# ds4dm/Tulip.jl

Hardware: AMD Instinct MI355X
Metric: IPM Newton-step rate: KKT.update! (A*D*A'+Rd, supernodal Cholesky) + 4 KKT.solve! (higher is better)
Workload: dtype f64

## Files before the change

### tulip.jl_amd/csrc/kernels.hip

```cpp
#include <hip/hip_runtime.h>

#include <algorithm>
#include <cstdlib>
#include <mutex>

#include "tlpk_device.hpp"

namespace tlpk {


typedef double v4f64 __attribute__((ext_vector_type(4)));
__device__ __forceinline__ double readlane_f64(const double v, const int l) {
    const int lo = __builtin_amdgcn_readlane(__double2loint(v), l), hi = __builtin_amdgcn_readlane(__double2hiint(v), l);
    return __hiloint2double(hi, lo);
}

__device__ __forceinline__ double *front_u(const DevCtx &c, const FrontDesc &fd) {
    return (fd.ubuf ? c.U1 : c.U0) + fd.uoff;
}
__device__ __forceinline__ double *pcol(const DevCtx &c, const FrontDesc &fd, i32 col) { return c.Lval + fd.loff + pk_off(fd.lda, col); }
__device__ __forceinline__ i32 pld(const FrontDesc &fd, i32 col) { return fd.lda - ((col >> 6) << 6); }
__device__ __forceinline__ bool front_skipped(const DevCtx &c, i32 front) { return c.front_skip != nullptr && c.front_skip[front] != 0; }
__device__ __forceinline__ void record_fail(const DevCtx &c, i32 col) {
    atomicMin(c.info, col);
// ... 129 lines not shown
                if (((tc - t.j0) & 3) != wave) continue;
                const double *__restrict__ src = Uc + (i64)q * rsc;
                double *__restrict__ dst = (tc < ns) ? pcol(c, fd, tc) : (Up + (i64)(tc - ns) * rs - ns);
                for (i32 r = max(q, rlo) + lane; r < rhi; r += 256) {
                    i32 tg[4]; double v[4], d[4];
#pragma unroll
                    for (int u = 0; u < 4; ++u) {
                        const i32 ru = min(r + 64 * u, rhi - 1);
                        tg[u] = relc[ru]; v[u] = src[ru];
                    }
#pragma unroll
                    for (int u = 0; u < 4; ++u) d[u] = dst[tg[u]];
#pragma unroll
                    for (int u = 0; u < 4; ++u) if (r + 64 * u < rhi) dst[tg[u]] = d[u] + v[u];
                }
            }
        }
    }
}

constexpr int EG_LD = EG_CAP_MAX / 64, EG_EB = 8, EG_CH = 2;
struct EgBatch { const i32 *rl[EG_EB]; const double *sr[EG_EB]; i32 n[EG_EB]; };
__device__ __forceinline__ EgBatch eg_entries(const DevCtx &c, const i64 e, const i64 e1) {
    EgBatch b;
#pragma unroll
    for (int u = 0; u < EG_EB; ++u) {
        const EaGatherEnt g = c.eg_ent[min(e + u, e1 - 1)];
        b.rl[u] = c.rel + g.rel;
        b.sr[u] = (((g.src >> EG_UBUF_BIT) & 1) ? c.U1 : c.U0) + (g.src & (((i64)1 << EG_UBUF_BIT) - 1));
        b.n[u] = (e + u < e1) ? g.n : 0;
    }
    return b;
}
__device__ __forceinline__ i32 eg_nmax(const EgBatch &b) {
    i32 m = 0;
#pragma unroll
    for (int u = 0; u < EG_EB; ++u) m = max(m, b.n[u]);
    return m;
}
__global__ __launch_bounds__(256, 4) void k_ea_gather(const EaTask *__restrict__ tasks, DevCtx c, int slice_rows) {
    extern __shared__ double eg_slices[];
    const EaTask t = tasks[blockIdx.x];
    if (!ea_task_gathered(c, t) || front_skipped(c, t.front)) return;
    const FrontDesc fd = c.fronts[t.front];
    const i32 f = fd.f, ns = fd.ns, rs = f - ns, cap = c.eg_cap;
    const int lane = threadIdx.x & 63;
    const int wave = __builtin_amdgcn_readfirstlane(threadIdx.x >> 6);
    double *slice = eg_slices + (size_t)wave * slice_rows;
    const i64 *colseg = c.eg_col + c.eg_base[t.front];
    double *Up = front_u(c, fd);
    for (i32 tc = t.j0 + wave; tc < t.j1; tc += 4) {
        double *__restrict__ col0 = (tc < ns) ? pcol(c, fd, tc) : (Up + (i64)(tc - ns) * rs - ns);
        const i64 g0 = colseg[tc], g1 = colseg[tc + 1];
        for (i64 g = g0; g < g1; ++g) {
            const i64 e0 = c.eg_ptr[g], e1 = c.eg_ptr[g + 1];
            if (e0 == e1) continue;
            const i32 r0 = tc + (i32)(g - g0) * cap, n = min(cap, f - r0);
            if (n > slice_rows) continue;
            double *__restrict__ col = col0 + r0;
            EgBatch b = eg_entries(c, e0, e1);
            double cv[EG_LD];
#pragma unroll
            for (int u = 0; u < EG_LD; ++u) cv[u] = col[min(lane + 64 * u, n - 1)];
            bool seeded = false;
            for (i64 e = e0; e < e1; e += EG_EB) {
                const bool thin = eg_nmax(b) <= 64 * EG_CH;
                i32 tg[EG_EB][EG_CH]; double v[EG_EB][EG_CH];
                if (thin) {
#pragma unroll
                    for (int u = 0; u < EG_EB; ++u)
#pragma unroll
                        for (int k = 0; k < EG_CH; ++k) {
                            const i32 ru = max(min(lane + 64 * k, b.n[u] - 1), 0);
                            tg[u][k] = b.rl[u][ru] - r0; v[u][k] = b.sr[u][ru];
                        }
                }
                if (!seeded) {
#pragma unroll
                    for (int u = 0; u < EG_LD; ++u) if (lane + 64 * u < n) slice[lane + 64 * u] = cv[u];
                    seeded = true;
                }
                EgBatch nb = b;
                if (e + EG_EB < e1) nb = eg_entries(c, e + EG_EB, e1);
                __builtin_amdgcn_wave_barrier();
                if (thin) {
#pragma unroll
                    for (int u = 0; u < EG_EB; ++u) {
                        double d[EG_CH];
#pragma unroll
                        for (int k = 0; k < EG_CH; ++k) d[k] = slice[tg[u][k]];
#pragma unroll
                        for (int k = 0; k < EG_CH; ++k) if (lane + 64 * k < b.n[u]) slice[tg[u][k]] = d[k] + v[u][k];
                        __builtin_amdgcn_wave_barrier();
                    }
                } else {
                    for (int u = 0; u < EG_EB; ++u) {
                        const i32 nu = b.n[u];
                        for (i32 r = lane; r - lane < nu; r += 256) {
                            i32 tq[4]; double w[4], d[4];
#pragma unroll
                            for (int k = 0; k < 4; ++k) { const i32 ru = min(r + 64 * k, nu - 1); tq[k] = b.rl[u][ru] - r0; w[k] = b.sr[u][ru]; }
#pragma unroll
                            for (int k = 0; k < 4; ++k) d[k] = slice[tq[k]];
#pragma unroll
                            for (int k = 0; k < 4; ++k) if (r + 64 * k < nu) slice[tq[k]] = d[k] + w[k];
                            __builtin_amdgcn_wave_barrier();
                        }
                    }
                }
                b = nb;
            }
            __builtin_amdgcn_wave_barrier();
            for (i32 r = lane; r < n; r += 64) col[r] = slice[r];
            __builtin_amdgcn_wave_barrier();
        }
    }
// ... 3417 lines not shown
    if (nrhs == 2) {
        if (L.kind == LK_FWD_SWEEP) {
            if (sw && L.pad) hipLaunchKernelGGL((k_fwd_sweep<2, true>), g, dim3(256), 0, st, a.fwd_sweep_tasks + L.first, a.ctx, *sw);
            else if (sw) hipLaunchKernelGGL(k_fwd_sweep<2>, g, dim3(256), 0, st, a.fwd_sweep_tasks + L.first, a.ctx, *sw);
            return;
        }
        if (L.kind == LK_BWD_SWEEP) {
            if (sw && L.pad) hipLaunchKernelGGL((k_bwd_sweep<2, true>), g, dim3(256), 0, st, a.bwd_sweep_tasks + L.first, a.ctx, *sw);
            else if (sw) hipLaunchKernelGGL(k_bwd_sweep<2>, g, dim3(256), 0, st, a.bwd_sweep_tasks + L.first, a.ctx, *sw);
            return;
        }
        const dim3 g2((unsigned)L.count, 2u);
        switch (L.kind) {
        case LK_FWD_GATHER: hipLaunchKernelGGL(k_fwd_gather, g2, dim3(256), 0, st, a.fwd_gather_tasks + L.first, a.ctx); return;
        case LK_FWD_SMALL: hipLaunchKernelGGL(k_fwd_small, g2, dim3(256), 0, st, a.fwd_small_tasks + L.first, a.ctx); return;
        case LK_BWD_SMALL: hipLaunchKernelGGL(k_bwd_small, g2, dim3(256), 0, st, a.bwd_small_tasks + L.first, a.ctx); return;
        default: break;
        }
        launch_tasks(st, a, L, sw, 1);
        DevArrays b = a;
        b.ctx.xw += a.ctx.xw2; b.ctx.uc += a.ctx.uc2;
        launch_tasks(st, b, L, sw, 1);
        return;
    }
#define TLPK_LAUNCH_S(KERNEL, TASKS) do { if (sgn) hipLaunchKernelGGL(KERNEL<true>, g, dim3(256), 0, st, TASKS + L.first, a.ctx); \
                                          else hipLaunchKernelGGL(KERNEL<false>, g, dim3(256), 0, st, TASKS + L.first, a.ctx); } while (0)
    switch (L.kind) {
    case LK_EXTEND_ADD: {
        static const unsigned ea_lds = [] { const char *e = std::getenv("TLPK_EA_LDS"); return e ? (unsigned)std::atoi(e) : 0u; }();
        bool plain = true;
        if (a.eg_launch) {
            const EaGatherLaunch *e = std::lower_bound(a.eg_launch, a.eg_launch + a.n_eg_launch, L.first, [](const EaGatherLaunch &x, i64 first) { return x.first < first; });
            if (e != a.eg_launch + a.n_eg_launch && e->first == L.first) {
                if (e->n_gather > 0)
                    hipLaunchKernelGGL(k_ea_gather, g, dim3(256), (unsigned)(4 * 8 * e->rows), st, a.ea_tasks + L.first, a.ctx, (int)e->rows);
                plain = e->n_plain > 0;
            }
        }
        if (plain) hipLaunchKernelGGL(k_extend_add, g, dim3(256), ea_lds, st, a.ea_tasks + L.first, a.ctx);
        break;
    }
    case LK_FRONT_ASSEMBLE:
        hipLaunchKernelGGL(k_front_assemble, g, dim3(256), 0, st, a.fa_tasks + L.first, a.ctx, a.asm_colptr, a.asm_target, a.asm_diag, a.asm_ptr,
                           a.pair_w, a.pair_j, a.asm_D, a.asm_regD);
        break;
    case LK_POTRF: case LK_POTRF_WIDE: {
        auto mode = [] {
            const char *m = std::getenv("TLPK_POTRF_MODE"); if (m) return std::atoi(m) & 3;
            const char *w = std::getenv("TLPK_POTRF_WAVE"); if (w && std::atoi(w) != 0) return 1;
            const char *e = std::getenv("TLPK_POTRF_PAIR"); if (e) return std::atoi(e) == 0 ? 0 : 2;
            return 3;
        };
        const bool dyn = std::getenv("TLPK_POTRF_DYN") != nullptr;
        static const int pm0 = mode();
        const int pm = dyn ? mode() : pm0;
#define TLPK_LAUNCH_PM(KERNEL, SG) do { if (pm == 3) hipLaunchKernelGGL((KERNEL<SG, 3>), g, dim3(256), 0, st, a.potrf_tasks + L.first, a.ctx); \
                                        else if (pm == 1) hipLaunchKernelGGL((KERNEL<SG, 1>), g, dim3(256), 0, st, a.potrf_tasks + L.first, a.ctx); \
                                        else if (pm == 2) hipLaunchKernelGGL((KERNEL<SG, 2>), g, dim3(256), 0, st, a.potrf_tasks + L.first, a.ctx); \
                                        else hipLaunchKernelGGL((KERNEL<SG, 0>), g, dim3(256), 0, st, a.potrf_tasks + L.first, a.ctx); } while (0)
#define TLPK_LAUNCH_P(KERNEL) do { if (sgn) TLPK_LAUNCH_PM(KERNEL, true); else TLPK_LAUNCH_PM(KERNEL, false); } while (0)
        if (L.kind == LK_POTRF) TLPK_LAUNCH_P(k_potrf); else TLPK_LAUNCH_P(k_potrf_wide);
#undef TLPK_LAUNCH_PM
#undef TLPK_LAUNCH_P
        break;
    }
    case LK_POTRF_SMALL: TLPK_LAUNCH_S(k_potrf_small, a.potrf_tasks); break;
    case LK_TRSM: TLPK_LAUNCH_S(k_trsm, a.trsm_tasks); break;
    case LK_TRSM_THIN: TLPK_LAUNCH_S(k_trsm_thin, a.trsm_tasks); break;
// ... 164 lines not shown
```

### tulip.jl_amd/csrc/symbolic.cpp

```cpp
#include "tlpk_host.hpp"
#include "schedule.hpp"
#include "../../include/tlpk.h"

#include <algorithm>
#include <atomic>
#include <thread>
#include <chrono>
#include <cstdio>
#include <array>
#include <cstdio>
#include <cstdlib>
#include <cstring>
#include <numeric>
#include <mutex>
#include <functional>
#include <condition_variable>
#include <map>
#include <climits>

namespace tlpk {

static inline i32 fa_min_f() {
    static const i32 v = [] { const char *e = std::getenv("TLPK_FA_MIN_F"); const int c = e ? std::atoi(e) : 0; return (i32)(c <= 0 ? INT32_MAX : c); }();
    return v;
// ... 1171 lines not shown
                i64 acc = 0;
                for (i64 e = a; e < b; ++e) { acc += S.pair_ptr[(size_t)e + 1]; S.pair_ptr[(size_t)e + 1] = acc; }
                tot[(size_t)ch + 1] = acc;
            });
            for (i64 ch = 0; ch < nch; ++ch) tot[(size_t)ch + 1] += tot[(size_t)ch];
            ok = ok && parallel_for(nch, host_threads(nch), [&](unsigned, i64 ch) {
                const i64 a = ch * CH, b = std::min(S.nnzS, a + CH), add = tot[(size_t)ch];
                if (add) for (i64 e = a; e < b; ++e) S.pair_ptr[(size_t)e + 1] += add;
            });
            if (!ok) return fail(S, TLPK_OOM, "out of memory while building the assembly lists");
            S.pair_ptr[0] = 0;
        }
        pt.mark("assembly lists: place");
        {
            S.pair_w.resize((size_t)S.pair_ptr[S.nnzS]); S.pair_j.resize((size_t)S.pair_ptr[S.nnzS]);
            const bool ok = parallel_for(m, host_threads(m / 256 + 1), [&](unsigned, i64 kk) {
                const i32 th = col_thr[(size_t)kk];
                if (th < 0) return;
                const i64 a = S.pair_ptr[(size_t)S.Sp[kk]], cnt = S.pair_ptr[(size_t)S.Sp[kk + 1]] - a;
                if (cnt <= 0) return;
                std::memcpy(S.pair_w.data() + a, st[(size_t)th].w.data() + col_off[(size_t)kk], (size_t)cnt * sizeof(double));
                std::memcpy(S.pair_j.data() + a, st[(size_t)th].j.data() + col_off[(size_t)kk], (size_t)cnt * sizeof(i32));
            }, 256);
            if (!ok) return fail(S, TLPK_OOM, "out of memory while building the assembly lists");
        }
    }
    pt.mark("schedule");
    S.error.clear();
    S.shared_device = opt.shared_device;
    build_schedule(S);
    if (!S.error.empty()) return TLPK_INTERNAL;
    for (const UpdateTask &u : S.update_tasks)
        if ((u.k0 & 15) != 0) return fail(S, TLPK_INTERNAL, "update task: K range does not start on a multiple of 16 columns");
    pt.mark(nullptr);
    return TLPK_OK;
}

int analyse(Symbolic &S, i64 m, i64 n, const i64 *colptr, const i64 *rowval, const double *nzval, int base, const Options &opt) {
    const int rc = analyse_common(S, m, n, colptr, rowval, nzval, base, opt);
    return rc != TLPK_OK ? rc : analyse_rank(S, opt);
}

int analyse_k2_common(Symbolic &S, i64 m, i64 n, const i64 *colptr, const i64 *rowval, const double *nzval,
                      int base, const Options &opt_in, Options *opt_out) {
    if (m < 0 || n < 0 || (base != 0 && base != 1) || !colptr) return fail(S, TLPK_BADARG, "bad dimensions or index base");
    if (opt_in.ordering == TLPK_ORDER_USER) return fail(S, TLPK_BADARG, "user_perm is not supported for K2");
    const i64 nnz = colptr[n] - base;
    if (nnz < 0 || m + n >= ((i64)1 << 31) || nnz >= ((i64)1 << 30)) return fail(S, TLPK_TOO_LARGE, "augmented system exceeds int32");
    if (nnz > 0 && (!rowval || !nzval)) return fail(S, TLPK_BADARG, "null rowval/nzval");
    std::vector<i64> bp((size_t)nnz + 1), bi((size_t)(2 * nnz));
    std::vector<double> bx((size_t)(2 * nnz));
    for (i64 j = 0; j < n; ++j) {
        if (colptr[j] - base < 0 || colptr[j + 1] < colptr[j] || colptr[j + 1] - base > nnz) return fail(S, TLPK_BADARG, "colptr not monotone");
        for (i64 p = colptr[j] - base; p < colptr[j + 1] - base; ++p) {
            const i64 r = rowval[p] - base;
            if (r < 0 || r >= m) return fail(S, TLPK_BADARG, "row index out of range");
            bp[(size_t)p] = 2 * p;
            bi[(size_t)(2 * p)] = j; bx[(size_t)(2 * p)] = 1.0;
            bi[(size_t)(2 * p + 1)] = n + r; bx[(size_t)(2 * p + 1)] = nzval[p];
        }
    }
    bp[(size_t)nnz] = 2 * nnz;
    Options opt = opt_in;
    opt.system = 1; opt.k2_n = n;
    std::vector<i64> node_block;
    if (opt_in.row_block) {
// ... 309 lines not shown
```

### tulip.jl_amd/csrc/tlpk_api.cpp

```cpp
#include <hip/hip_runtime.h>

#include <dlfcn.h>

#include <algorithm>
#include <atomic>
#include <chrono>
#include <climits>
#include <cmath>
#include <limits>
#include <cstdio>
#include <cstdlib>
#include <cstring>
#include <new>
#include <optional>
#include <string>
#include <thread>
#include <utility>
#include <vector>
#include <condition_variable>
#include <functional>
#include <initializer_list>
#include <mutex>

#include "../../include/tlpk.h"
// ... 156 lines not shown
        Launch cur = L[i];
        if ((h->profile || h->serial) && cur.kind == LK_UPDATE) {
            if (skip_update == i) continue;
            if (cur.side) {
                for (size_t j = i + 1; j < to && L[j].kind != LK_SIDE_JOIN; ++j)
                    if (L[j].kind == LK_UPDATE && !L[j].side && L[j].first == cur.first + cur.count) {
                        cur.count += L[j].count; skip_update = j; break;
                    }
            }
        }
        const bool stag = h->stagger && dir < 0 && !h->profile && !h->serial && cur.kind == LK_EXTEND_ADD && h->S.ngroups >= 2 && h->ev_stagger;
        if (stag && L[i].group == 1 && h->stagger_armed) { hipStreamWaitEvent(st, h->ev_stagger, 0); h->stagger_armed = false; }
        ProfScope ps(h, kind_class(cur.kind), st, &cur);
        if (stag && L[i].group == 0 && cur.count >= h->stagger_min) {
            launch_tasks(st, h->d, cur, nullptr, nrhs);
            hipEventRecord(h->ev_stagger, st); h->stagger_armed = true;
            continue;
        }
        if (cur.kind == LK_FWD_SWEEP || cur.kind == LK_BWD_SWEEP) {
            const i32 slot = (dir == 0 ? h->sweep_slot_fwd : h->sweep_slot_bwd)[i];
            SweepArgs sw{h->d.sweep_tickets + slot, h->d.sweep_xh + (dir == 0 ? 0 : h->S.m), 2 * h->S.m, h->poll[0], h->poll[1], h->poll[2], dir == 0 ? h->d.fwd_small_tasks : h->d.bwd_small_tasks};
            launch_tasks(st, h->d, cur, &sw, nrhs);
        } else
            launch_tasks(st, h->d, cur, nullptr, nrhs);
    }
    join_groups(h);
}

std::vector<EaGatherLaunch> eg_count_launches(const Symbolic &S) {
    std::vector<EaGatherLaunch> out;
    if (S.ea_gather_ent.empty()) return out;
    for (const Launch &L : S.factor_launches) {
        if (L.kind != LK_EXTEND_ADD || L.count <= 0) continue;
        EaGatherLaunch g{L.first, 0, 0, 1};
        for (i64 k = L.first; k < L.first + L.count; ++k) {
            const EaTask &t = S.ea_tasks[(size_t)k];
            if (S.ea_gather_base[(size_t)t.front] >= 0 && t.br1 == 0) { g.n_gather++; g.rows = std::max(g.rows, std::min(S.fronts[(size_t)t.front].f - t.j0, S.ea_gather_cap)); }
            else g.n_plain++;
        }
        if (g.n_gather > 0) out.push_back(g);
    }
    return out;
}

int upload_all(tlpk_handle *h) {
    Symbolic &S = h->S;
    DevArrays &d = h->d;
    d.m = S.m; d.n = S.n;
    d.mu = (S.system == 1) ? S.k2_m : S.m - S.n_dense;
    const i64 mu = d.mu;
    int rc;
#define UP(dst, vec) if ((rc = dev_upload(h, &(dst), (vec))) != TLPK_OK) return rc
    if (S.dense_matrix) {
        d.dlda = dense_lda(S.m);
        d.syrk_split = S.syrk_split;
        d.syrk_kc = S.syrk_kc;
        d.gemv_chunks = S.gemv_chunks;
        d.gemv_cw = std::max<i64>(1, (S.n + S.gemv_chunks - 1) / S.gemv_chunks);
        if ((rc = dev_alloc(h, &d.gemv_part, 2 * S.gemv_chunks * d.dlda)) != TLPK_OK) return rc;
    }
    UP(d.Ap, S.Ap); UP(d.Ai, S.Ai); UP(d.Ax, S.Ax);
    UP(d.Tp, S.Tp); UP(d.Tj, S.Tj);
    {
        std::vector<double> Tx(S.Tpos.size());
        for (size_t q = 0; q < Tx.size(); ++q) Tx[q] = S.Ax[S.Tpos[q]];
        UP(d.Tx, Tx);
    }
    UP(d.perm, S.perm);
    if (S.system == 0 && !S.dense_matrix) {
        std::vector<i64> Pp((size_t)S.m + 1, 0);
// ... 56 lines not shown
                    if (S.front_fa[(size_t)S.sn_of_col[(size_t)kk]])
                        for (i64 q = colptr[(size_t)kk]; q < colptr[(size_t)kk + 1]; ++q) tsmall[(size_t)q] = -1;
                UP(d.asm_colptr, colptr); UP(d.asm_target_small, tsmall);
            }
            bool any = false;
            for (char f : S.front_upper) any |= (f != 0);
            d.has_upper = any;
            if (any) {
                std::vector<unsigned char> up((size_t)d.n_asm, 0);
                for (i64 kk = 0; kk < S.m; ++kk)
                    if (S.front_upper[(size_t)S.sn_of_col[(size_t)kk]]) std::fill(up.begin() + colptr[(size_t)kk], up.begin() + colptr[(size_t)kk + 1], (unsigned char)1);
                UP(d.asm_upper, up);
            }
        }
        if (every) { UP(d.asm_target, S.s_target); UP(d.asm_diag, S.s_diag_row); UP(d.asm_ptr, S.pair_ptr); }
        else { UP(d.asm_target, tgt); UP(d.asm_diag, diag); UP(d.asm_ptr, ptr); }
        if (!d.asm_target_small) d.asm_target_small = d.asm_target;
        UP(d.pair_w, S.pair_w); UP(d.pair_j, S.pair_j);
        if (np != (i64)S.pair_w.size()) { h->last_error = "assembly list compaction mismatch"; return TLPK_INTERNAL; }
    }
    const FrontDesc *fr = nullptr; const i32 *ri = nullptr, *re = nullptr, *ch = nullptr;
    { FrontDesc *p; UP(p, S.fronts); fr = p; }
    { i32 *p; UP(p, S.rowidx); ri = p; }
    { i32 *p; UP(p, S.rel); re = p; }
    { i32 *p; UP(p, S.ea_tab); d.ctx.ea_tab = p; }
    { i32 *p; UP(p, S.children); ch = p; }
    d.ctx.fronts = fr; d.ctx.rowidx = ri; d.ctx.rel = re; d.ctx.children = ch;
    { i64 *p; UP(p, S.gth_ptr); d.ctx.gth_ptr = p; }
    { i64 *p; UP(p, S.gth_src); d.ctx.gth_src = p; }
    UP(d.fa_tasks, S.fa_tasks);
    UP(d.ea_tasks, S.ea_tasks); UP(d.potrf_tasks, S.potrf_tasks); UP(d.trsm_tasks, S.trsm_tasks);
    if (!S.ea_gather_ent.empty()) {
        std::vector<unsigned char> gf(S.fronts.size(), 0);
        for (size_t s = 0; s < gf.size(); ++s) gf[s] = S.ea_gather_base[s] >= 0;
        { unsigned char *p; UP(p, gf); d.ctx.eg_front = p; }
        { i64 *p; UP(p, S.ea_gather_base); d.ctx.eg_base = p; }
        { i64 *p; UP(p, S.ea_gather_col); d.ctx.eg_col = p; }
        { i64 *p; UP(p, S.ea_gather_ptr); d.ctx.eg_ptr = p; }
        { EaGatherEnt *p; UP(p, S.ea_gather_ent); d.ctx.eg_ent = p; }
        d.ctx.eg_cap = S.ea_gather_cap;
        h->eg_launches = eg_count_launches(S);
        if (!h->eg_launches.empty()) { d.eg_launch = h->eg_launches.data(); d.n_eg_launch = (i64)h->eg_launches.size(); }
        else d.ctx.eg_front = nullptr;
    }
    UP(d.update_tasks, S.update_tasks); UP(d.reduce_tasks, S.reduce_tasks);
    UP(d.chain_items, S.chain_items); d.n_chain_cnt = S.chain_counters;
    if (S.chain_counters > 0 && (rc = dev_alloc(h, &d.chain_cnt, S.chain_counters)) != TLPK_OK) return rc;
    if (!S.chain_items.empty() && std::getenv("TLPK_CHAIN_TRACE") && (rc = dev_alloc(h, &d.chain_trace, 4 * (i64)S.chain_items.size())) != TLPK_OK) return rc;
    { i32 *p; UP(p, S.upd_seg); d.ctx.upd_seg = p; }
    d.n_single = (i64)S.single_col.size();
    UP(d.single_loff, S.single_loff); UP(d.single_dinvoff, S.single_dinvoff); UP(d.single_col, S.single_col);
    UP(d.zero_tasks, S.zero_tasks); d.n_zero_tasks = (i64)S.zero_tasks.size() / 2; d.n_zero_lower = d.has_upper ? S.n_zero_lower : d.n_zero_tasks;
    UP(d.zero_small, S.zero_small); d.n_zero_small = (i64)S.zero_small.size();
    UP(d.fwd_gather_tasks, S.fwd_gather_tasks); UP(d.fwd_diag_tasks, S.fwd_diag_tasks);
    UP(d.fwd_update_tasks, S.fwd_update_tasks); UP(d.bwd_update_tasks, S.bwd_update_tasks);
    UP(d.fwd_small_tasks, S.fwd_small_tasks); UP(d.bwd_small_tasks, S.bwd_small_tasks);
    UP(d.fwd_sweep_tasks, S.fwd_sweep_tasks); UP(d.bwd_sweep_tasks, S.bwd_sweep_tasks);
#undef UP
#define AL(dst, cnt) if ((rc = dev_alloc(h, &(dst), (cnt))) != TLPK_OK) return rc
    AL(d.ctx.Lval, S.lval_len); AL(d.ctx.U0, S.ubuf_len[0]); AL(d.ctx.U1, S.ubuf_len[1]);
    if (std::getenv("TLPK_POISON") && S.lval_len > 0) { HIPCHK(h, hipMemset(d.ctx.Lval, 0xFF, (size_t)S.lval_len * 8)); HIPCHK(h, hipDeviceSynchronize()); }
    AL(d.ctx.uc, 2 * S.uc_len); AL(d.ctx.xw, 2 * S.m); AL(d.ctx.info, INFO_WORDS + S.m);
    d.ctx.xw2 = S.m; d.ctx.uc2 = S.uc_len; AL(d.ctx.dinv, S.dinv_len); AL(d.ctx.spart, S.spart_len);
    const i64 nn = std::max<i64>(S.n + (S.n_dense > 0 ? 1 : 0), S.k2_n + 1);
    AL(h->d_theta, nn); AL(h->d_regP, nn); AL(h->d_regD, S.m); AL(h->d_D, nn);
    AL(h->d_xip, S.m); AL(h->d_xid, nn); AL(h->d_dx, nn); AL(h->d_dy, S.m);
    AL(d.rhs_w, std::max<i64>(2 * S.n, 1));
    d.asm_D = h->d_D; d.asm_regD = h->d_regD;
    HIPCHK(h, hipMemset(h->d_theta, 0, (size_t)nn * 8)); HIPCHK(h, hipMemset(h->d_regP, 0, (size_t)nn * 8)); HIPCHK(h, hipMemset(h->d_xid, 0, (size_t)nn * 8));
    HIPCHK(h, hipMemset(h->d_regD, 0, (size_t)std::max<i64>(S.m, 1) * 8)); HIPCHK(h, hipMemset(h->d_xip, 0, (size_t)std::max<i64>(S.m, 1) * 8));
    if (h->refine_steps > 0) { AL(h->d_r1, S.m); AL(h->d_r2, nn); AL(h->d_cx, nn); AL(h->d_cy, S.m); AL(h->d_ref, 8); }
    d.ctx.csign = nullptr;
    d.ctx.small_full = std::getenv("TLPK_SMALL_FULL") ? std::atoi(std::getenv("TLPK_SMALL_FULL")) : 0;
    d.ctx.upd_remap = 2;
    if (const char *e = std::getenv("TLPK_UPD_REMAP")) d.ctx.upd_remap = std::atoi(e);
    if (S.system == 1 || S.n_dense > 0) { double *p; if ((rc = dev_upload(h, &p, S.csign)) != TLPK_OK) return rc; d.ctx.csign = p; }
#undef AL
    {
        i32 nslots = 0;
        h->sweep_slot_fwd.assign(S.fwd_launches.size(), -1); h->sweep_slot_bwd.assign(S.bwd_launches.size(), -1);
        for (size_t i = 0; i < S.fwd_launches.size(); ++i) if (S.fwd_launches[i].kind == LK_FWD_SWEEP) h->sweep_slot_fwd[i] = nslots++;
        for (size_t i = 0; i < S.bwd_launches.size(); ++i) if (S.bwd_launches[i].kind == LK_BWD_SWEEP) h->sweep_slot_bwd[i] = nslots++;
        const i64 nt = ((i64)nslots + 15) / 16 * 16;
        unsigned long long *blk = nullptr;
        if ((rc = dev_alloc(h, &blk, nt + 4 * S.m)) != TLPK_OK) return rc;
        d.sweep_tickets = blk; d.sweep_xh = reinterpret_cast<double *>(blk + nt);
// ... 2197 lines not shown
    }
    const i64 mu = user_m(h);
    i64 o = 0;
    for (i64 i = 0; i < h->S.m; ++i) if (h->S.system == 1 || h->S.perm[(size_t)i] < mu) perm[o++] = h->S.perm[(size_t)i];
    return TLPK_OK;
}

int64_t tlpk_symbolic_get(const tlpk_handle *h, const char *what, int64_t *buf, int64_t cap) {
    if (!h || !what) return -1;
    if (!h->sub.empty() && std::string(what) != "chain_retries") return tlpk_symbolic_get(h->sub[0], what, buf, cap);
    const Symbolic &S = h->S;
    std::vector<i64> tmp;
    const std::string w(what);
    auto from32 = [&](const auto &v) { tmp.assign(v.begin(), v.end()); };
    auto field = [&](auto getter) { tmp.resize(S.fronts.size()); for (size_t s = 0; s < S.fronts.size(); ++s) tmp[s] = (i64)getter(S.fronts[s]); };
    if (w == "perm") from32(S.perm);
    else if (w == "etree") from32(S.parent);
    else if (w == "colcount") from32(S.colcount);
    else if (w == "s_colptr") tmp = S.Sp;
    else if (w == "s_rowidx") from32(S.Si);
    else if (w == "s_target") from32(S.s_target);
    else if (w == "s_diag_row") from32(S.s_diag_row);
    else if (w == "pair_ptr") from32(S.pair_ptr);
    else if (w == "pair_j") from32(S.pair_j);
    else if (w == "rowidx") from32(S.rowidx);
    else if (w == "rel") from32(S.rel);
    else if (w == "ea_tab") from32(S.ea_tab);
    else if (w == "ea_gather_base") tmp = S.ea_gather_base;
    else if (w == "ea_gather_col") tmp = S.ea_gather_col;
    else if (w == "ea_gather_ptr") tmp = S.ea_gather_ptr;
    else if (w == "ea_gather_ent") { for (auto &g : S.ea_gather_ent) { tmp.push_back(g.src); tmp.push_back(g.rel); tmp.push_back(g.n); tmp.push_back(g.child); } }
    else if (w == "ea_gather_cap") tmp.assign(1, S.ea_gather_cap);
    else if (w == "ea_gather_launches") { for (auto &g : eg_count_launches(S)) { tmp.push_back(g.first); tmp.push_back(g.n_gather); tmp.push_back(g.n_plain); tmp.push_back(g.rows); } }
    else if (w == "front_eatab") field([](const FrontDesc &f) { return f.eatab; });
    else if (w == "children") from32(S.children);
    else if (w == "depth") from32(S.depth);
    else if (w == "front_block") from32(S.front_block);
    else if (w == "row_block") tmp = h->row_block_copy;
    else if (w == "front_group") from32(S.front_group);
    else if (w == "ngroups") tmp.assign(1, S.ngroups);
    else if (w == "front_local") tmp.assign(S.front_local.begin(), S.front_local.end());
    else if (w == "col_local") tmp.assign(S.col_local.begin(), S.col_local.end());
    else if (w == "row_local") tmp.assign(S.row_local.begin(), S.row_local.end());
    else if (w == "front_f") field([](const FrontDesc &f) { return f.f; });
    else if (w == "front_lda") field([](const FrontDesc &f) { return f.lda; });
    else if (w == "front_ns") field([](const FrontDesc &f) { return f.ns; });
    else if (w == "front_col0") field([](const FrontDesc &f) { return f.col0; });
    else if (w == "front_parent") field([](const FrontDesc &f) { return f.parent; });
    else if (w == "front_loff") field([](const FrontDesc &f) { return f.loff; });
    else if (w == "front_rowoff") field([](const FrontDesc &f) { return f.rowoff; });
    else if (w == "front_reloff") field([](const FrontDesc &f) { return f.reloff; });
    else if (w == "front_child_ptr") field([](const FrontDesc &f) { return f.child_ptr; });
    else if (w == "front_nchild") field([](const FrontDesc &f) { return f.nchild; });
    else if (w == "root_front") tmp.assign(1, S.root_front);
    else if (w == "dense_cols") tmp = S.dense_cols;
    else if (w == "potrf_tasks") { for (auto &t : S.potrf_tasks) { tmp.push_back(t.front); tmp.push_back(t.k0); tmp.push_back(t.nb); tmp.push_back(t.kprev); } }
    else if (w == "trsm_tasks") { for (auto &t : S.trsm_tasks) { tmp.push_back(t.front); tmp.push_back(t.k0); tmp.push_back(t.nb); tmp.push_back(t.row0); tmp.push_back(t.kprev); tmp.push_back(t.pad1); } }
    else if (w == "update_tasks") { for (auto &t : S.update_tasks) { tmp.push_back(t.front); tmp.push_back(t.k0); tmp.push_back(t.kw); tmp.push_back(t.i0); tmp.push_back(t.j0); tmp.push_back(t.jlim); tmp.push_back(t.beta0); tmp.push_back(t.pad1); tmp.push_back(t.seg); tmp.push_back(t.nsl); } }
    else if (w == "upd_seg") from32(S.upd_seg);
    else if (w == "trsm_early") { for (auto &t : S.trsm_tasks) tmp.push_back(t.pad2); }
    else if (w == "update_tile64") { for (auto &t : S.update_tasks) tmp.push_back(t.pad2); }
    else if (w == "skip_off") tmp = S.skip_off;
    else if (w == "skip_bits") { tmp.resize(S.skip_bits.size()); std::memcpy(tmp.data(), S.skip_bits.data(), S.skip_bits.size() * 8); }
    else if (w == "front_single") tmp.assign(S.front_single.begin(), S.front_single.end());
    else if (w == "reduce_tasks") { for (auto &t : S.reduce_tasks) { tmp.push_back(t.front); tmp.push_back(t.k0); tmp.push_back(t.kw); tmp.push_back(t.i0); tmp.push_back(t.j0); tmp.push_back(t.jlim); tmp.push_back(t.beta0); tmp.push_back(t.pad1); } }
    else if (w == "chain_items") { for (auto &t : S.chain_items) { for (i32 v : {t.role, t.task, t.sub, t.w0, t.n0, t.need0, t.w1, t.n1, t.need1, t.w2, t.need2, t.sig}) tmp.push_back(v); } }
// ... 102 lines not shown
```

### tulip.jl_amd/csrc/tlpk_device.hpp

```cpp
#pragma once
#include <hip/hip_runtime.h>

#include "tlpk_host.hpp"

namespace tlpk {

struct DevCtx {
    const FrontDesc *fronts;
    const i32 *rowidx;
    const i32 *rel;
    const i32 *ea_tab;
    const i32 *children;
    const i64 *gth_ptr, *gth_src;
    double *Lval;
    double *U0, *U1;
    double *uc;
    double *xw;
    double *dinv;
    double *spart;
    int *info;
    int upd_remap;
    const double *csign;
    const i32 *upd_seg;
    int small_full;
    i64 xw2, uc2;
    const unsigned char *eg_front; const i64 *eg_base, *eg_col, *eg_ptr; const EaGatherEnt *eg_ent; i32 eg_cap;
    const unsigned char *front_skip;
};
constexpr int INFO_WORDS = 16;

struct SweepArgs {
    unsigned long long *ticket;
    double *xh;
    i64 xh2;
    int poll_fast, poll_nfast, poll_slow;
    const SolveTask *small = nullptr;
};

struct EaGatherLaunch { i64 first; i32 n_gather, n_plain, rows; };

struct DevArrays {
    DevCtx ctx{};
    const EaGatherLaunch *eg_launch = nullptr; i64 n_eg_launch = 0;
    i64 m = 0, n = 0;
    i64 mu = 0;
    char *sparse_col = nullptr; i32 *dense_col = nullptr; i64 n_dense = 0;
    const double *dA = nullptr; i64 dlda = 0;
    i32 syrk_split = 1; i64 syrk_kc = 0;
    double *gemv_part = nullptr; i64 gemv_chunks = 0, gemv_cw = 0;
    i64 *Ap = nullptr; i32 *Ai = nullptr; double *Ax = nullptr;
    i64 *Tp = nullptr; i32 *Tj = nullptr; double *Tx = nullptr;
    i32 *perm = nullptr;
    i64 *Pp = nullptr; i32 *Pj = nullptr; double *Px = nullptr;
    double *rhs_w = nullptr;
    i32 *zero_tasks = nullptr; i64 n_zero_tasks = 0;
    i64 n_zero_lower = 0;
    unsigned char *asm_upper = nullptr; bool has_upper = false;
    i32 *zero_small = nullptr; i64 n_zero_small = 0;
    char *row_local = nullptr, *col_local = nullptr;
    i64 n_asm = 0;
    i64 *asm_target = nullptr; i32 *asm_diag = nullptr; i64 *asm_ptr = nullptr;
    double *pair_w = nullptr; i32 *pair_j = nullptr;
    FaTask *fa_tasks = nullptr;
    i64 *asm_colptr = nullptr;
    i64 *asm_target_small = nullptr;
    const double *asm_D = nullptr, *asm_regD = nullptr;
    EaTask *ea_tasks = nullptr; PotrfTask *potrf_tasks = nullptr; TrsmTask *trsm_tasks = nullptr;
    UpdateTask *update_tasks = nullptr, *reduce_tasks = nullptr;
    ChainItem *chain_items = nullptr;
    unsigned long long *chain_trace = nullptr;
    unsigned *chain_cnt = nullptr; i64 n_chain_cnt = 0;
    i64 n_single = 0; i64 *single_loff = nullptr, *single_dinvoff = nullptr; i32 *single_col = nullptr;
    SolveTask *fwd_gather_tasks = nullptr, *fwd_diag_tasks = nullptr, *fwd_update_tasks = nullptr,
              *bwd_update_tasks = nullptr, *fwd_small_tasks = nullptr, *bwd_small_tasks = nullptr,
              *fwd_sweep_tasks = nullptr, *bwd_sweep_tasks = nullptr;
    unsigned long long *sweep_tickets = nullptr;
// ... 136 lines not shown
```

### tulip.jl_amd/csrc/tlpk_host.hpp

```cpp
#pragma once
#include <cstdint>
#include <string>
#include <vector>

namespace tlpk {

using i32 = int32_t;
using i64 = int64_t;

constexpr int NB_IN = 64;
constexpr int NB_OUT = 256;
constexpr int TILE = 128;
constexpr int TRSM_ROWS = 64;
constexpr int SMALL_NS = 16;
constexpr int SMALL_ROWS = 256;
constexpr int TRSM_THIN_W = 32;
constexpr int TRSM_WG_ROWS = 64;
constexpr int EA_COLS = 16;
constexpr int SOLVE_NB = 128;
constexpr int SWEEP_NB = NB_IN;
constexpr int MAX_GROUPS = 8;
constexpr int LDA_PAD_MIN_F = 64;
constexpr int SOLVE_ROWS = 256;
constexpr int GATHER_WIDE_PER_ROW = 16;
// ... 82 lines not shown
        if constexpr (sizeof...(A) == 0) ::new (static_cast<void *>(p)) U; else ::new (static_cast<void *>(p)) U(std::forward<A>(a)...);
    }
};
template <class T> using uvec = std::vector<T, NoInit<T>>;

struct Symbolic {
    i64 m = 0, n = 0, nnzA = 0;
    i32 system = 0; i64 k2_n = 0, k2_m = 0;
    i32 shared_device = 0;
    std::vector<double> csign;
    i64 n_dense = 0, dense_n = 0;
    i32 dense_matrix = 0;
    i64 syrk_slots = 0;
    i32 syrk_split = 1;
    i64 syrk_kc = 16;
    i64 gemv_chunks = 0;
    double flops_syrk = 0;
    std::vector<i64> dense_cols;
    std::vector<i64> Ap; std::vector<i32> Ai; std::vector<double> Ax;
    std::vector<i64> Tp; std::vector<i32> Tj; std::vector<i32> Tpos;
    std::vector<i32> Acol;
    std::vector<i32> perm, iperm;
    std::vector<i64> Sp; std::vector<i32> Si;
    std::vector<i32> parent;
    std::vector<i32> colcount;
    i32 nsuper = 0;
    std::vector<FrontDesc> fronts;
    std::vector<i32> sn_of_col;
    std::vector<i32> rowidx;
    std::vector<i32> rel;
    std::vector<i32> ea_tab;
    std::vector<i64> ea_gather_base, ea_gather_col, ea_gather_ptr; std::vector<EaGatherEnt> ea_gather_ent;
    i32 ea_gather_cap = 0;
    std::vector<i64> gth_ptr, gth_src;
    std::vector<i32> children;
    std::vector<i32> depth;
    i32 nlevels = 0;
    std::vector<i32> level_ptr, level_fronts;
    i32 nblocks = 0;
    std::vector<i32> front_block;
    std::vector<char> front_local;
    std::vector<char> front_single;
    std::vector<i64> single_loff, single_dinvoff; std::vector<i32> single_col;
    std::vector<i32> zero_tasks;
    std::vector<i32> zero_small;
    std::vector<char> front_upper;
    i64 n_zero_lower = 0;
    std::vector<char> col_local;
    std::vector<char> row_local;
    i32 root_front = -1;
    i32 ngroups = 1;
    std::vector<i32> front_group;
    i32 n_local_blocks = 0;
    uvec<i64> s_target;
    uvec<i32> s_diag_row;
    uvec<i64> pair_ptr;
    uvec<double> pair_w;
    uvec<i32> pair_j;
    uvec<char> s_local;
    i64 nnzS = 0, nnzL = 0, lval_len = 0, ubuf_len[2] = {0, 0}, uc_len = 0, max_front = 0, dinv_len = 0;
    double flops_chol = 0, flops_panel = 0, flops_update = 0, flops_update_alg = 0;
    double flops_update_chain = 0, flops_update_alg_chain = 0;
    std::vector<PotrfTask> potrf_tasks; std::vector<TrsmTask> trsm_tasks;
    std::vector<UpdateTask> update_tasks, reduce_tasks; std::vector<EaTask> ea_tasks;
    std::vector<FaTask> fa_tasks;
    std::vector<char> front_fa;
// ... 46 lines not shown
```

Measured before the change: 20.91.

## Form eligible fronts inside extend-add gather, skipping separate zeroing pass

```diff
diff --git a/tulip.jl_amd/csrc/kernels.hip b/tulip.jl_amd/csrc/kernels.hip
--- a/tulip.jl_amd/csrc/kernels.hip
+++ b/tulip.jl_amd/csrc/kernels.hip
@@ -185,18 +185,48 @@
     }
     return b;
 }
+__device__ __forceinline__ i64 eg_rl64(const i64 v, const int l) {
+    const unsigned lo = (unsigned)__builtin_amdgcn_readlane((int)(unsigned)v, l), hi = (unsigned)__builtin_amdgcn_readlane((int)(v >> 32), l);
+    return (i64)(((unsigned long long)hi << 32) | lo);
+}
+__device__ __forceinline__ EgBatch eg_entries_lanes(const DevCtx &c, const i64 e, const i64 e1, const int lane) {
+    const EaGatherEnt g = c.eg_ent[max(min(e + (lane & (EG_EB - 1)), e1 - 1), (i64)0)];
+    EgBatch b;
+#pragma unroll
+    for (int u = 0; u < EG_EB; ++u) {
+        const i64 src = eg_rl64(g.src, u), rel = eg_rl64(g.rel, u);
+        b.rl[u] = c.rel + rel;
+        b.sr[u] = (((src >> EG_UBUF_BIT) & 1) ? c.U1 : c.U0) + (src & (((i64)1 << EG_UBUF_BIT) - 1));
+        b.n[u] = (e + u < e1) ? __builtin_amdgcn_readlane(g.n, u) : 0;
+    }
+    return b;
+}
 __device__ __forceinline__ i32 eg_nmax(const EgBatch &b) {
     i32 m = 0;
 #pragma unroll
     for (int u = 0; u < EG_EB; ++u) m = max(m, b.n[u]);
     return m;
 }
-__global__ __launch_bounds__(256, 4) void k_ea_gather(const EaTask *__restrict__ tasks, DevCtx c, int slice_rows) {
+constexpr int EG_AL = 2;
+__device__ __forceinline__ void eg_put_formed(const unsigned short *__restrict__ asm_row, double *slice, const double *col, const double (&av)[EG_AL], const i32 (&arow)[EG_AL], const i64 a0, const i32 na,
+                                              const i32 n, const int lane) {
+#pragma unroll
+    for (int u = 0; u < EG_LD; ++u) if (lane + 64 * u < n) slice[lane + 64 * u] = 0.0;
+    __builtin_amdgcn_wave_barrier();
+#pragma unroll
+    for (int k = 0; k < EG_AL; ++k) if (lane + 64 * k < na) slice[arow[k]] = av[k];
+    for (i32 i = 64 * EG_AL + lane; i < na; i += 64) { const i32 r = asm_row[a0 + i]; slice[r] = col[r]; }
+}
+__device__ __forceinline__ bool ea_task_formed(const DevCtx &c, const EaTask &t, const i32 ns) { return (c.eg_front[t.front] & EG_FORMED) != 0 && t.j0 < ns; }
+template <bool FORM>
+__global__ __launch_bounds__(256, 4) void k_ea_gather(const EaTask *__restrict__ tasks, DevCtx c, int slice_rows, const i64 *__restrict__ asm_ptr,
+                                                      const unsigned short *__restrict__ asm_row) {
     extern __shared__ double eg_slices[];
     const EaTask t = tasks[blockIdx.x];
     if (!ea_task_gathered(c, t) || front_skipped(c, t.front)) return;
     const FrontDesc fd = c.fronts[t.front];
     const i32 f = fd.f, ns = fd.ns, rs = f - ns, cap = c.eg_cap;
+    if (ea_task_formed(c, t, ns) != FORM) return;
     const int lane = threadIdx.x & 63;
     const int wave = __builtin_amdgcn_readfirstlane(threadIdx.x >> 6);
     double *slice = eg_slices + (size_t)wave * slice_rows;
@@ -205,18 +235,39 @@
     for (i32 tc = t.j0 + wave; tc < t.j1; tc += 4) {
         double *__restrict__ col0 = (tc < ns) ? pcol(c, fd, tc) : (Up + (i64)(tc - ns) * rs - ns);
         const i64 g0 = colseg[tc], g1 = colseg[tc + 1];
+        if constexpr (FORM) {
+            for (i32 r = (tc & ~63) + lane; r < tc; r += 64) col0[r] = 0.0;
+            for (i32 r = f + lane; r < fd.lda; r += 64) col0[r] = 0.0;
+        }
         for (i64 g = g0; g < g1; ++g) {
             const i64 e0 = c.eg_ptr[g], e1 = c.eg_ptr[g + 1];
-            if (e0 == e1) continue;
+            if (!FORM && e0 == e1) continue;
             const i32 r0 = tc + (i32)(g - g0) * cap, n = min(cap, f - r0);
             if (n > slice_rows) continue;
             double *__restrict__ col = col0 + r0;
-            EgBatch b = eg_entries(c, e0, e1);
-            double cv[EG_LD];
-#pragma unroll
-            for (int u = 0; u < EG_LD; ++u) cv[u] = col[min(lane + 64 * u, n - 1)];
+            i32 na = 0; i64 a0 = 0;
+            i32 arow[EG_AL] = {}; double av[EG_AL] = {};
+            if constexpr (FORM) {
+                a0 = asm_ptr[g];
+                na = (i32)(asm_ptr[g + 1] - a0);
+                if (na > 0) {
+#pragma unroll
+                    for (int k = 0; k < EG_AL; ++k) arow[k] = asm_row[a0 + min(lane + 64 * k, na - 1)];
+                }
+            }
+            EgBatch b = FORM ? eg_entries_lanes(c, e0, e1, lane) : eg_entries(c, e0, e1);
+            double cv[FORM ? 1 : EG_LD];
+            if constexpr (FORM) {
+                if (na > 0) {
+#pragma unroll
+                    for (int k = 0; k < EG_AL; ++k) av[k] = col[arow[k]];
+                }
+            } else {
+#pragma unroll
+                for (int u = 0; u < EG_LD; ++u) cv[u] = col[min(lane + 64 * u, n - 1)];
+            }
             bool seeded = false;
-            for (i64 e = e0; e < e1; e += EG_EB) {
+            for (i64 e = e0; e < e1 || (FORM && !seeded); e += EG_EB) {
                 const bool thin = eg_nmax(b) <= 64 * EG_CH;
                 i32 tg[EG_EB][EG_CH]; double v[EG_EB][EG_CH];
                 if (thin) {
@@ -229,12 +280,15 @@
                         }
                 }
                 if (!seeded) {
-#pragma unroll
-                    for (int u = 0; u < EG_LD; ++u) if (lane + 64 * u < n) slice[lane + 64 * u] = cv[u];
+                    if constexpr (FORM) eg_put_formed(asm_row, slice, col, av, arow, a0, na, n, lane);
+                    else {
+#pragma unroll
+                        for (int u = 0; u < EG_LD; ++u) if (lane + 64 * u < n) slice[lane + 64 * u] = cv[u];
+                    }
                     seeded = true;
                 }
                 EgBatch nb = b;
-                if (e + EG_EB < e1) nb = eg_entries(c, e + EG_EB, e1);
+                if (e + EG_EB < e1) nb = FORM ? eg_entries_lanes(c, e + EG_EB, e1, lane) : eg_entries(c, e + EG_EB, e1);
                 __builtin_amdgcn_wave_barrier();
                 if (thin) {
 #pragma unroll
@@ -3718,8 +3772,11 @@
         if (a.eg_launch) {
             const EaGatherLaunch *e = std::lower_bound(a.eg_launch, a.eg_launch + a.n_eg_launch, L.first, [](const EaGatherLaunch &x, i64 first) { return x.first < first; });
             if (e != a.eg_launch + a.n_eg_launch && e->first == L.first) {
-                if (e->n_gather > 0)
-                    hipLaunchKernelGGL(k_ea_gather, g, dim3(256), (unsigned)(4 * 8 * e->rows), st, a.ea_tasks + L.first, a.ctx, (int)e->rows);
+                if (e->n_gather > e->n_form)
+                    hipLaunchKernelGGL(k_ea_gather<false>, g, dim3(256), (unsigned)(4 * 8 * e->rows), st, a.ea_tasks + L.first, a.ctx, (int)e->rows, (const i64 *)nullptr,
+                                       (const unsigned short *)nullptr);
+                if (e->n_form > 0)
+                    hipLaunchKernelGGL(k_ea_gather<true>, g, dim3(256), (unsigned)(4 * 8 * e->rows), st, a.ea_tasks + L.first, a.ctx, (int)e->rows, a.eg_asm_ptr, a.eg_asm_row);
                 plain = e->n_plain > 0;
             }
         }
diff --git a/tulip.jl_amd/csrc/symbolic.cpp b/tulip.jl_amd/csrc/symbolic.cpp
--- a/tulip.jl_amd/csrc/symbolic.cpp
+++ b/tulip.jl_amd/csrc/symbolic.cpp
@@ -1227,6 +1227,56 @@
     if (!S.error.empty()) return TLPK_INTERNAL;
     for (const UpdateTask &u : S.update_tasks)
         if ((u.k0 & 15) != 0) return fail(S, TLPK_INTERNAL, "update task: K range does not start on a multiple of 16 columns");
+    S.ea_form.clear(); S.ea_gather_asm_ptr.clear(); S.ea_gather_asm_row.clear();
+    {
+        bool on = true;
+        if (const char *e = std::getenv("TLPK_EA_FORM")) on = std::atoi(e) != 0;
+        const size_t nf = S.fronts.size();
+        std::vector<unsigned char> form(nf, 0);
+        bool any = false;
+        if (on && !S.ea_gather_ent.empty()) {
+            std::vector<i64> covered(nf, 0);
+            std::vector<char> banded(nf, 0);
+            for (const EaTask &t : S.ea_tasks) {
+                if (S.ea_gather_base[(size_t)t.front] < 0) continue;
+                if (t.br1 != 0) banded[(size_t)t.front] = 1;
+                else if (t.j1 <= S.fronts[(size_t)t.front].ns) covered[(size_t)t.front] += t.j1 - t.j0;
+            }
+            for (size_t s = 0; s < nf; ++s)
+                if (S.ea_gather_base[s] >= 0 && !S.front_fa[s] && !banded[s] && covered[s] == S.fronts[s].ns) { form[s] = 1; any = true; }
+        }
+        if (any) {
+            const i32 cap = S.ea_gather_cap;
+            const i64 nseg = (i64)S.ea_gather_ptr.size() - 1;
+            std::vector<i64> &ptr = S.ea_gather_asm_ptr;
+            ptr.assign((size_t)nseg + 1, 0);
+            for (int pass = 0; pass < 2; ++pass) {
+                std::vector<i64> fill;
+                if (pass == 1) {
+                    for (i64 g = 0; g < nseg; ++g) ptr[(size_t)g + 1] += ptr[(size_t)g];
+                    S.ea_gather_asm_row.assign((size_t)ptr[(size_t)nseg], 0);
+                    fill.assign(ptr.begin(), ptr.end() - 1);
+                }
+                for (size_t s = 0; s < nf; ++s) {
+                    if (!form[s]) continue;
+                    const FrontDesc &w = S.fronts[s];
+                    const i64 *colseg = S.ea_gather_col.data() + S.ea_gather_base[s];
+                    for (i32 tc = 0; tc < w.ns; ++tc) {
+                        const i64 kk = (i64)w.col0 + tc, vrow0 = w.loff + pk_off(w.lda, tc);
+                        for (i64 e = S.Sp[(size_t)kk]; e < S.Sp[(size_t)kk + 1]; ++e) {
+                            const i64 row = S.s_target[(size_t)e] - vrow0;
+                            if (!S.s_local[(size_t)e] || row < tc || row >= w.f) return fail(S, TLPK_INTERNAL, "formed front: an assembly target outside its panel column");
+                            const i64 pc = (row - tc) / cap, g = colseg[tc] + pc;
+                            if (pass == 0) ptr[(size_t)g + 1]++;
+                            else S.ea_gather_asm_row[(size_t)fill[(size_t)g]++] = (uint16_t)(row - tc - pc * cap);
+                        }
+                    }
+                }
+            }
+            for (i64 g = 0; g < nseg; ++g) std::sort(S.ea_gather_asm_row.begin() + ptr[(size_t)g], S.ea_gather_asm_row.begin() + ptr[(size_t)g + 1]);
+            S.ea_form = std::move(form);
+        }
+    }
     pt.mark(nullptr);
     return TLPK_OK;
 }
diff --git a/tulip.jl_amd/csrc/tlpk_api.cpp b/tulip.jl_amd/csrc/tlpk_api.cpp
--- a/tulip.jl_amd/csrc/tlpk_api.cpp
+++ b/tulip.jl_amd/csrc/tlpk_api.cpp
@@ -212,10 +212,13 @@
     if (S.ea_gather_ent.empty()) return out;
     for (const Launch &L : S.factor_launches) {
         if (L.kind != LK_EXTEND_ADD || L.count <= 0) continue;
-        EaGatherLaunch g{L.first, 0, 0, 1};
+        EaGatherLaunch g{L.first, 0, 0, 1, 0};
         for (i64 k = L.first; k < L.first + L.count; ++k) {
             const EaTask &t = S.ea_tasks[(size_t)k];
-            if (S.ea_gather_base[(size_t)t.front] >= 0 && t.br1 == 0) { g.n_gather++; g.rows = std::max(g.rows, std::min(S.fronts[(size_t)t.front].f - t.j0, S.ea_gather_cap)); }
+            if (S.ea_gather_base[(size_t)t.front] >= 0 && t.br1 == 0) {
+                g.n_gather++; g.rows = std::max(g.rows, std::min(S.fronts[(size_t)t.front].f - t.j0, S.ea_gather_cap));
+                if (!S.ea_form.empty() && S.ea_form[(size_t)t.front] && t.j0 < S.fronts[(size_t)t.front].ns) g.n_form++;
+            }
             else g.n_plain++;
         }
         if (g.n_gather > 0) out.push_back(g);
@@ -338,7 +341,7 @@
     UP(d.ea_tasks, S.ea_tasks); UP(d.potrf_tasks, S.potrf_tasks); UP(d.trsm_tasks, S.trsm_tasks);
     if (!S.ea_gather_ent.empty()) {
         std::vector<unsigned char> gf(S.fronts.size(), 0);
-        for (size_t s = 0; s < gf.size(); ++s) gf[s] = S.ea_gather_base[s] >= 0;
+        for (size_t s = 0; s < gf.size(); ++s) gf[s] = S.ea_gather_base[s] < 0 ? 0 : (unsigned char)(EG_GATHERED | (!S.ea_form.empty() && S.ea_form[s] ? EG_FORMED : 0));
         { unsigned char *p; UP(p, gf); d.ctx.eg_front = p; }
         { i64 *p; UP(p, S.ea_gather_base); d.ctx.eg_base = p; }
         { i64 *p; UP(p, S.ea_gather_col); d.ctx.eg_col = p; }
@@ -348,6 +351,10 @@
         h->eg_launches = eg_count_launches(S);
         if (!h->eg_launches.empty()) { d.eg_launch = h->eg_launches.data(); d.n_eg_launch = (i64)h->eg_launches.size(); }
         else d.ctx.eg_front = nullptr;
+        if (d.ctx.eg_front && !S.ea_form.empty()) {
+            { i64 *p; UP(p, S.ea_gather_asm_ptr); d.eg_asm_ptr = p; }
+            { uint16_t *p; UP(p, S.ea_gather_asm_row); d.eg_asm_row = p; }
+        }
     }
     UP(d.update_tasks, S.update_tasks); UP(d.reduce_tasks, S.reduce_tasks);
     UP(d.chain_items, S.chain_items); d.n_chain_cnt = S.chain_counters;
@@ -356,8 +363,21 @@
     { i32 *p; UP(p, S.upd_seg); d.ctx.upd_seg = p; }
     d.n_single = (i64)S.single_col.size();
     UP(d.single_loff, S.single_loff); UP(d.single_dinvoff, S.single_dinvoff); UP(d.single_col, S.single_col);
-    UP(d.zero_tasks, S.zero_tasks); d.n_zero_tasks = (i64)S.zero_tasks.size() / 2; d.n_zero_lower = d.has_upper ? S.n_zero_lower : d.n_zero_tasks;
-    UP(d.zero_small, S.zero_small); d.n_zero_small = (i64)S.zero_small.size();
+    if (d.eg_asm_ptr) {
+        std::vector<i32> zt, zs;
+        i64 lower = 0;
+        for (size_t k = 0; k + 1 < S.zero_tasks.size(); k += 2) {
+            if (S.ea_form[(size_t)S.zero_tasks[k]]) continue;
+            zt.push_back(S.zero_tasks[k]); zt.push_back(S.zero_tasks[k + 1]);
+            if ((i64)k / 2 < S.n_zero_lower) ++lower;
+        }
+        for (const i32 s : S.zero_small) if (!S.ea_form[(size_t)s]) zs.push_back(s);
+        UP(d.zero_tasks, zt); d.n_zero_tasks = (i64)zt.size() / 2; d.n_zero_lower = d.has_upper ? lower : d.n_zero_tasks;
+        UP(d.zero_small, zs); d.n_zero_small = (i64)zs.size();
+    } else {
+        UP(d.zero_tasks, S.zero_tasks); d.n_zero_tasks = (i64)S.zero_tasks.size() / 2; d.n_zero_lower = d.has_upper ? S.n_zero_lower : d.n_zero_tasks;
+        UP(d.zero_small, S.zero_small); d.n_zero_small = (i64)S.zero_small.size();
+    }
     UP(d.fwd_gather_tasks, S.fwd_gather_tasks); UP(d.fwd_diag_tasks, S.fwd_diag_tasks);
     UP(d.fwd_update_tasks, S.fwd_update_tasks); UP(d.bwd_update_tasks, S.bwd_update_tasks);
     UP(d.fwd_small_tasks, S.fwd_small_tasks); UP(d.bwd_small_tasks, S.bwd_small_tasks);
@@ -2621,6 +2641,9 @@
     else if (w == "ea_gather_ent") { for (auto &g : S.ea_gather_ent) { tmp.push_back(g.src); tmp.push_back(g.rel); tmp.push_back(g.n); tmp.push_back(g.child); } }
     else if (w == "ea_gather_cap") tmp.assign(1, S.ea_gather_cap);
     else if (w == "ea_gather_launches") { for (auto &g : eg_count_launches(S)) { tmp.push_back(g.first); tmp.push_back(g.n_gather); tmp.push_back(g.n_plain); tmp.push_back(g.rows); } }
+    else if (w == "ea_form") tmp.assign(S.ea_form.begin(), S.ea_form.end());
+    else if (w == "ea_gather_asm_ptr") tmp = S.ea_gather_asm_ptr;
+    else if (w == "ea_gather_asm_row") tmp.assign(S.ea_gather_asm_row.begin(), S.ea_gather_asm_row.end());
     else if (w == "front_eatab") field([](const FrontDesc &f) { return f.eatab; });
     else if (w == "children") from32(S.children);
     else if (w == "depth") from32(S.depth);
diff --git a/tulip.jl_amd/csrc/tlpk_device.hpp b/tulip.jl_amd/csrc/tlpk_device.hpp
--- a/tulip.jl_amd/csrc/tlpk_device.hpp
+++ b/tulip.jl_amd/csrc/tlpk_device.hpp
@@ -27,6 +27,7 @@
     const unsigned char *eg_front; const i64 *eg_base, *eg_col, *eg_ptr; const EaGatherEnt *eg_ent; i32 eg_cap;
     const unsigned char *front_skip;
 };
+constexpr unsigned char EG_GATHERED = 1, EG_FORMED = 2;
 constexpr int INFO_WORDS = 16;
 
 struct SweepArgs {
@@ -37,11 +38,12 @@
     const SolveTask *small = nullptr;
 };
 
-struct EaGatherLaunch { i64 first; i32 n_gather, n_plain, rows; };
+struct EaGatherLaunch { i64 first; i32 n_gather, n_plain, rows, n_form; };
 
 struct DevArrays {
     DevCtx ctx{};
     const EaGatherLaunch *eg_launch = nullptr; i64 n_eg_launch = 0;
+    const i64 *eg_asm_ptr = nullptr; const unsigned short *eg_asm_row = nullptr;
     i64 m = 0, n = 0;
     i64 mu = 0;
     char *sparse_col = nullptr; i32 *dense_col = nullptr; i64 n_dense = 0;
diff --git a/tulip.jl_amd/csrc/tlpk_host.hpp b/tulip.jl_amd/csrc/tlpk_host.hpp
--- a/tulip.jl_amd/csrc/tlpk_host.hpp
+++ b/tulip.jl_amd/csrc/tlpk_host.hpp
@@ -138,6 +138,7 @@
     std::vector<i32> ea_tab;
     std::vector<i64> ea_gather_base, ea_gather_col, ea_gather_ptr; std::vector<EaGatherEnt> ea_gather_ent;
     i32 ea_gather_cap = 0;
+    std::vector<unsigned char> ea_form; std::vector<i64> ea_gather_asm_ptr; std::vector<uint16_t> ea_gather_asm_row;
     std::vector<i64> gth_ptr, gth_src;
     std::vector<i32> children;
     std::vector<i32> depth;
```

New measurement: 21.30, median of 6. 1.8% higher.
